# PaddlePaddle/PaddleNLP

Hardware: AMD Instinct MI355X
Metric: tokens_per_sec_whole_node_llama3_8b_pretrain (higher is better)
Workload: dtype bf16; 1 GPU; model=llama3-8b, global_batch=8, seq_len=4096, parallelism=single, recompute=False

## Files before the change

paddlenlp_amd/ops/csrc/flash_attn_bwd_v2.hip:

```cpp
#include "launchers.h"
#include "mfma.h"

#define FB2_WAVES 8
#define FB2_BLOCK (FB2_WAVES * 64)

template <int D, bool MASKED = false>
__global__ __launch_bounds__(FB2_BLOCK) void flash_bwd2_dq_kernel(
    const ushort_t* __restrict__ q, const ushort_t* __restrict__ k,
    const ushort_t* __restrict__ v, const ushort_t* __restrict__ dout,
    const float* __restrict__ lse, const float* __restrict__ delta,
    ushort_t* __restrict__ dq, const int* __restrict__ startend,
    FlashStrides rs,
    int B, int Sq, int Skv, int Hq, int Hk, float scale, int causal) {
    static_assert(D == 128, "the dual-use image is laid out for 128-column tiles");
    constexpr int BLKN = 64;
    constexpr int DSTEPS = D / 16;
    constexpr int NDT = D / 32;
    constexpr int BLKM = FB2_WAVES * 32;

    __shared__ __attribute__((aligned(16))) ushort_t kv_lds[2][2][BLKN * D];
    __shared__ int se_lds[3][MASKED ? BLKN : 1];

    const int tid = threadIdx.x;
    const int wave = __builtin_amdgcn_readfirstlane(tid >> 6);
    const int lane = tid & 63;
    const int l32 = lane & 31;
    const int hi = lane >> 5;

    int qt, bh;
    xcd_grouped_tile<FA_ORDER_W, false>(qt, bh);
    const int b = bh / Hq, hq = bh % Hq;
    const int hk = hq / (Hq / Hk);
    const int q_base = qt * BLKM;
    const int qw = q_base + wave * 32;
    const int qg = qw + l32;
    const int causal_off = Skv - Sq;

    const long long q_row_stride = rs.q;
    const long long kv_row_stride = rs.kv;
    const long long do_row_stride = (long long)Hq * D;
    const ushort_t* q_ptr = q + (long long)b * Sq * q_row_stride + (long long)hq * D;
    const ushort_t* do_ptr = dout + ((long long)b * Sq * Hq + hq) * D;
    const ushort_t* k_ptr = k + (long long)b * Skv * kv_row_stride + (long long)hk * D;
    const ushort_t* v_ptr = v + (long long)b * Skv * kv_row_stride + (long long)hk * D;

    frag8 aq[DSTEPS], ado[DSTEPS];
    float lse_q = INFINITY, dl_q = 0.f;
    if (qg < Sq) {
#pragma unroll
        for (int kk = 0; kk < DSTEPS; kk++) {
            aq[kk] = *reinterpret_cast<const frag8*>(
                q_ptr + (long long)qg * q_row_stride + kk * 16 + hi * 8);
            ado[kk] = *reinterpret_cast<const frag8*>(
                do_ptr + (long long)qg * do_row_stride + kk * 16 + hi * 8);
        }
        lse_q = lse[((long long)b * Hq + hq) * Sq + qg];
        dl_q = delta[((long long)b * Hq + hq) * Sq + qg];
    } else {
#pragma unroll
        for (int kk = 0; kk < DSTEPS; kk++) { aq[kk] = frag8{0}; ado[kk] = frag8{0}; }
    }

    f32x16 acc_dq[NDT];
#pragma unroll
    for (int n = 0; n < NDT; n++)
#pragma unroll
        for (int r = 0; r < 16; r++) acc_dq[n][r] = 0.f;

    int n_kv_tiles = (Skv + BLKN - 1) / BLKN;
    if (causal) {
        int max_kv = q_base + BLKM - 1 + causal_off;
        int lim = (max_kv + BLKN) / BLKN;
        n_kv_tiles = min(n_kv_tiles, max(lim, 0));
    }

    auto issue_tile = [&](int kv_base, int buf) {
        const int ln = fresh_lane_id();
#pragma unroll
        for (int i = 0; i < 2; i++) {
            const int piece = wave * 2 + i;
            const int src_row = min(kv_base + img_fill_row(piece, ln), Skv - 1);
            const long long off = (long long)src_row * kv_row_stride +
                                  img_fill_chunk(piece, ln) * 8;
            lds_dma16(k_ptr + off, &kv_lds[buf][0][piece * 512]);
            lds_dma16(v_ptr + off, &kv_lds[buf][1][piece * 512]);
        }
    };
    auto issue_bounds = [&](int tile, int slot) {
        if (MASKED && wave == 0) {
            const int ln = fresh_lane_id();
            lds_dma4(startend + (long long)b * Skv + min(tile * BLKN + ln, Skv - 1),
                     &se_lds[slot][0]);
        }
    };
    auto tile_se_max = [&](int slot) -> int {
        int v = se_lds[slot][lane];
#pragma unroll
        for (int off = 32; off; off >>= 1)
            v = max(v, __shfl_xor(v, off, 64));
        return __builtin_amdgcn_readfirstlane(v);
    };

#pragma unroll
    for (int kk = 0; kk < DSTEPS; kk++)
        asm volatile("" :: "v"(aq[kk]), "v"(ado[kk]));
    asm volatile("" :: "v"(lse_q), "v"(dl_q));
    if (n_kv_tiles > 0) {
        issue_tile(0, 0);
        issue_bounds(0, 0);
        if (n_kv_tiles > 1) issue_bounds(1, 1);
    }
    int se_max_cur = 0x7fffffff;
    int se_slot = 0;

    for (int kvt = 0; kvt < n_kv_tiles; kvt++) {
        const int kv_base = kvt * BLKN;
        const int cur = kvt & 1;
        lds_dma_wait_all();
        __syncthreads();
        const int se_slot_next = (se_slot == 2) ? 0 : se_slot + 1;
        if (MASKED && kvt == 0) se_max_cur = tile_se_max(0);
        int se_max_next = 0x7fffffff;
        if (kvt + 1 < n_kv_tiles) {
            bool stage_skip = false;
            if (MASKED) {
                se_max_next = tile_se_max(se_slot_next);
                stage_skip = (q_base >= se_max_next);
            }
            if (!stage_skip) issue_tile(kv_base + BLKN, cur ^ 1);
            if (kvt + 2 < n_kv_tiles)
                issue_bounds(kvt + 2, (se_slot_next == 2) ? 0 : se_slot_next + 1);
        }
        const ushort_t* k_img = kv_lds[cur][0];
        const ushort_t* v_img = kv_lds[cur][1];
        const int lane_t = fresh_lane_id();

        bool wave_skip =
            causal && (kv_base > qw + 31 + causal_off);
        if (MASKED && qw >= se_max_cur) wave_skip = true;

        auto process_sub = [&](int sub) {
            f32x16 st, dp;
#pragma unroll
            for (int r = 0; r < 16; r++) { st[r] = 0.f; dp[r] = 0.f; }
            __builtin_amdgcn_s_setprio(1);
#pragma unroll
            for (int kk = 0; kk < DSTEPS; kk++) {
                frag8 ak = img_row_frag(k_img, sub * 32 + l32, kk, hi);
                frag8 av = img_row_frag(v_img, sub * 32 + l32, kk, hi);
                st = mfma32(ak, aq[kk], st);
                dp = mfma32(av, ado[kk], dp);
            }
            __builtin_amdgcn_s_setprio(0);

#pragma unroll
            for (int r = 0; r < 16; r++) {
                int row = sub * 32 + crow32(r, hi);
                int kvg = kv_base + row;
                bool vis = (kvg < Skv) && (qg < Sq) &&
                           (!causal || kvg <= qg + causal_off);
                if (MASKED) vis = vis && (qg < se_lds[se_slot][row]);
                float p = vis ? __expf(st[r] * scale - lse_q) : 0.f;
                st[r] = p * (dp[r] - dl_q) * scale;
            }

            __builtin_amdgcn_s_setprio(1);
#pragma unroll
            for (int ksl = 0; ksl < 2; ksl++) {
                const int ks = sub * 2 + ksl;
                frag8 ads = t12_convert(st, ksl * 8);
#pragma unroll
                for (int n = 0; n < NDT; n++) {
                    frag8 bkf = img_tr_frag(k_img, ks, n, lane_t);
                    acc_dq[n] = mfma32(ads, bkf, acc_dq[n]);
                }
            }
            __builtin_amdgcn_s_setprio(0);
        };

        if (!wave_skip) {
            process_sub(0);
            process_sub(1);
        }
        if (MASKED) se_max_cur = se_max_next;
        se_slot = se_slot_next;
    }

#pragma unroll
    for (int r = 0; r < 16; r++) {
        int qrow = qw + crow32(r, hi);
        if (qrow >= Sq) continue;
        ushort_t* dqr = dq + ((long long)b * Sq + qrow) * rs.dq + (long long)hq * D;
#pragma unroll
        for (int n = 0; n < NDT; n++)
            dqr[n * 32 + l32] = f32_to_bf16(acc_dq[n][r]);
    }
}

template <int D, bool MASKED = false>
__global__ __launch_bounds__(FB2_BLOCK, 1) void flash_bwd2_dkv_kernel(
    const ushort_t* __restrict__ q, const ushort_t* __restrict__ k,
    const ushort_t* __restrict__ v, const ushort_t* __restrict__ dout,
    const float* __restrict__ lse, const float* __restrict__ delta,
    ushort_t* __restrict__ dk, ushort_t* __restrict__ dv,
    const int* __restrict__ startend,
    FlashStrides rs,
    int B, int Sq, int Skv, int Hq, int Hk, float scale, int causal) {
    static_assert(D == 128, "the dual-use image is laid out for 128-column tiles");
    constexpr int BLKQ = 64;
    constexpr int DSTEPS = D / 16;
    constexpr int NDT = D / 32;
    constexpr int BLKKV = FB2_WAVES * 32;

    __shared__ __attribute__((aligned(16))) ushort_t qd_lds[2][2][BLKQ * D];
    __shared__ float ld_lds[2][2][BLKQ];

    const int tid = threadIdx.x;
    const int wave = __builtin_amdgcn_readfirstlane(tid >> 6);
    const int lane = tid & 63;
    const int l32 = lane & 31;
    const int hi = lane >> 5;

    int kvt, bh;
    xcd_grouped_tile<FA_ORDER_W, true>(kvt, bh);
    const int b = bh / Hk, hk = bh % Hk;
    const int G = Hq / Hk;
    const int kv_base = kvt * BLKKV;
    const int kvw = kv_base + wave * 32;
    const int kvg_lane = kvw + l32;
    const int causal_off = Skv - Sq;
    __shared__ int blk_max_lds[MASKED ? FB2_WAVES : 1];
    int kv_end_lane = 0x7fffffff;
    int wave_max_end = 0x7fffffff;
    if (MASKED) {
        kv_end_lane = (kvg_lane < Skv)
            ? startend[(long long)b * Skv + kvg_lane] : 0;
        wave_max_end = kv_end_lane;
#pragma unroll
        for (int off = 32; off; off >>= 1)
            wave_max_end = max(wave_max_end,
                               __shfl_xor(wave_max_end, off, 64));
        wave_max_end = __builtin_amdgcn_readfirstlane(wave_max_end);
        if (lane == 0) blk_max_lds[wave] = wave_max_end;
    }

    const long long do_row_stride = (long long)Hq * D;
    const ushort_t* k_ptr = k + (long long)b * Skv * rs.kv + (long long)hk * D;
    const ushort_t* v_ptr = v + (long long)b * Skv * rs.kv + (long long)hk * D;

    frag8 bk[DSTEPS], bv[DSTEPS];
    if (kvg_lane < Skv) {
#pragma unroll
        for (int kk = 0; kk < DSTEPS; kk++) {
            bk[kk] = *reinterpret_cast<const frag8*>(
                k_ptr + (long long)kvg_lane * rs.kv + kk * 16 + hi * 8);
            bv[kk] = *reinterpret_cast<const frag8*>(
                v_ptr + (long long)kvg_lane * rs.kv + kk * 16 + hi * 8);
        }
    } else {
#pragma unroll
        for (int kk = 0; kk < DSTEPS; kk++) { bk[kk] = frag8{0}; bv[kk] = frag8{0}; }
    }

    f32x16 acc_dk[NDT], acc_dv[NDT];
#pragma unroll
    for (int n = 0; n < NDT; n++)
#pragma unroll
        for (int r = 0; r < 16; r++) { acc_dk[n][r] = 0.f; acc_dv[n][r] = 0.f; }

    int qt0 = 0;
    if (causal) qt0 = max(0, (kv_base - causal_off) / BLKQ);
    int qt_end = (Sq + BLKQ - 1) / BLKQ;
    if (MASKED) {
        __syncthreads();
        int block_max_end = blk_max_lds[0];
#pragma unroll
        for (int w = 1; w < FB2_WAVES; w++)
            block_max_end = max(block_max_end, blk_max_lds[w]);
        block_max_end = __builtin_amdgcn_readfirstlane(block_max_end);
        if (block_max_end < Sq)
            qt_end = (max(block_max_end, 0) + BLKQ - 1) / BLKQ;
    }
    const int n_tiles = G * max(qt_end - qt0, 0);

    auto issue_tile = [&](int g, int qt, int buf) {
        const int hq = hk * G + g;
        const long long do_off = ((long long)b * Sq * Hq + hq) * D;
        const long long q_off = (long long)b * Sq * rs.q + (long long)hq * D;
        const int q_tb = qt * BLKQ;
        const int ln = fresh_lane_id();
#pragma unroll
        for (int i = 0; i < 2; i++) {
            const int piece = wave * 2 + i;
            const int src_row = min(q_tb + img_fill_row(piece, ln), Sq - 1);
            const int chunk = img_fill_chunk(piece, ln) * 8;
            lds_dma16(q + (q_off + (long long)src_row * rs.q + chunk),
                      &qd_lds[buf][0][piece * 512]);
            lds_dma16(dout + (do_off + (long long)src_row * do_row_stride + chunk),
                      &qd_lds[buf][1][piece * 512]);
        }
        if (wave < 2) {
            const float* row = (wave == 0 ? lse : delta) +
                               ((long long)b * Hq + hq) * Sq;
            lds_dma4(row + min(q_tb + ln, Sq - 1), &ld_lds[buf][wave][0]);
        }
    };

    int g_next = 0, qt_next = qt0;
    auto advance_next = [&]() {
        if (++qt_next == qt_end) { qt_next = qt0; g_next++; }
    };
#pragma unroll
    for (int kk = 0; kk < DSTEPS; kk++)
        asm volatile("" :: "v"(bk[kk]), "v"(bv[kk]));
    if (n_tiles > 0) { issue_tile(g_next, qt_next, 0); advance_next(); }

    int qt = qt0;
    for (int t = 0; t < n_tiles; t++) {
        const int cur = t & 1;
        lds_dma_wait_all();
        __syncthreads();
        if (t + 1 < n_tiles) { issue_tile(g_next, qt_next, cur ^ 1); advance_next(); }

        const int q_tb = qt * BLKQ;
        const ushort_t* q_img = qd_lds[cur][0];
        const ushort_t* do_img = qd_lds[cur][1];
        const int lane_t = fresh_lane_id();
        bool wave_skip =
            causal && (q_tb + BLKQ - 1 + causal_off < kvw);
        if (MASKED && q_tb >= wave_max_end) wave_skip = true;

        if (!wave_skip) {
#pragma unroll 1
            for (int sub = 0; sub < 2; sub++) {
                f32x16 st, dp;
#pragma unroll
                for (int r = 0; r < 16; r++) { st[r] = 0.f; dp[r] = 0.f; }
                __builtin_amdgcn_s_setprio(1);
#pragma unroll
                for (int kk = 0; kk < DSTEPS; kk++) {
                    frag8 aqf = img_row_frag(q_img, sub * 32 + l32, kk, hi);
                    frag8 adf = img_row_frag(do_img, sub * 32 + l32, kk, hi);
                    st = mfma32(aqf, bk[kk], st);
                    dp = mfma32(adf, bv[kk], dp);
                }
                __builtin_amdgcn_s_setprio(0);

#pragma unroll
                for (int r = 0; r < 16; r++) {
                    int qrow = sub * 32 + crow32(r, hi);
                    int qgl = q_tb + qrow;
                    float ls = ld_lds[cur][0][qrow];
                    float dl = ld_lds[cur][1][qrow];
                    bool vis = (qgl < Sq) && (kvg_lane < Skv) &&
                               (!causal || kvg_lane <= qgl + causal_off);
                    if (MASKED) vis = vis && (qgl < kv_end_lane);
                    float p = (vis && ls != INFINITY)
                                  ? __expf(st[r] * scale - ls) : 0.f;
                    st[r] = p;
                    dp[r] = p * (dp[r] - dl) * scale;
                }

                __builtin_amdgcn_s_setprio(1);
#pragma unroll
                for (int ksl = 0; ksl < 2; ksl++) {
                    const int ks = sub * 2 + ksl;
                    frag8 apt = t12_convert(st, ksl * 8);
                    frag8 ads = t12_convert(dp, ksl * 8);
#pragma unroll
                    for (int n = 0; n < NDT; n++) {
                        frag8 bdo = img_tr_frag(do_img, ks, n, lane_t);
                        frag8 bq = img_tr_frag(q_img, ks, n, lane_t);
                        acc_dv[n] = mfma32(apt, bdo, acc_dv[n]);
                        acc_dk[n] = mfma32(ads, bq, acc_dk[n]);
                    }
                }
                __builtin_amdgcn_s_setprio(0);
            }
        }
        if (++qt == qt_end) qt = qt0;
    }

#pragma unroll
    for (int r = 0; r < 16; r++) {
        int kvr = kvw + crow32(r, hi);
        if (kvr >= Skv) continue;
        long long base = ((long long)b * Skv + kvr) * rs.dkv + (long long)hk * D;
#pragma unroll
        for (int n = 0; n < NDT; n++) {
            dk[base + n * 32 + l32] = f32_to_bf16(acc_dk[n][r]);
            dv[base + n * 32 + l32] = f32_to_bf16(acc_dv[n][r]);
        }
    }
}

__global__ __launch_bounds__(64) void lds_image_probe(
    const ushort_t* __restrict__ X, ushort_t* __restrict__ out_row,
    ushort_t* __restrict__ out_tr) {
    __shared__ __attribute__((aligned(16))) ushort_t img[64 * 128];
    const int lane = threadIdx.x;
    const int l32 = lane & 31, hi = lane >> 5;
#pragma unroll 1
    for (int piece = 0; piece < 16; piece++)
        lds_dma16(X + img_fill_row(piece, lane) * 128 + img_fill_chunk(piece, lane) * 8,
                  &img[piece * 512]);
    lds_dma_wait_all();
    __syncthreads();
    for (int sub = 0; sub < 2; sub++)
        for (int kk = 0; kk < 8; kk++) {
            frag8 f = img_row_frag(img, sub * 32 + l32, kk, hi);
            *reinterpret_cast<frag8*>(
                out_row + (sub * 32 + l32) * 128 + kk * 16 + hi * 8) = f;
        }
    for (int ks = 0; ks < 4; ks++)
        for (int n = 0; n < 4; n++) {
            frag8 f = img_tr_frag(img, ks, n, lane);
#pragma unroll
            for (int j = 0; j < 8; j++)
                out_tr[(ks * 16 + hi * 8 + j) * 128 + n * 32 + l32] = (ushort_t)f[j];
        }
}

void launch_lds_image_probe(const void* X, void* out_row, void* out_tr,
                            hipStream_t stream) {
    hipLaunchKernelGGL(lds_image_probe, dim3(1), dim3(64), 0, stream,
                       (const ushort_t*)X, (ushort_t*)out_row, (ushort_t*)out_tr);
}

bool launch_flash_bwd2(const void* dout, const void* q, const void* k, const void* v,
                       const void* o, const float* lse, float* delta,
                       void* dq, void* dk, void* dv,
                       int B, int Sq, int Skv, int Hq, int Hk, int D,
                       float scale, bool causal, hipStream_t stream, int parts,
                       const FlashStrides* strides) {
    if (D != 128 || (Hq % Hk) != 0) return false;
    const FlashStrides rs = strides ? *strides : flash_contiguous_strides(Hq, Hk, D);
    if (!flash_dma_aligned(q, rs.q) || !flash_dma_aligned(k, rs.kv) ||
        !flash_dma_aligned(v, rs.kv) || !flash_dma_aligned(dout, Hq * D))
        return false;
    if (parts & FLASH_BWD_DELTA)
        launch_flash_bwd_delta(dout, o, delta, B, Sq, Hq, D, stream);
    if (parts & FLASH_BWD_DQ) {
        dim3 gq((Sq + 255) / 256, B * Hq);
        hipLaunchKernelGGL((flash_bwd2_dq_kernel<128, false>), gq, dim3(FB2_BLOCK), 0, stream,
                           (const ushort_t*)q, (const ushort_t*)k, (const ushort_t*)v,
                           (const ushort_t*)dout, lse, delta, (ushort_t*)dq,
                           (const int*)nullptr, rs,
                           B, Sq, Skv, Hq, Hk, scale, causal ? 1 : 0);
    }
    if (parts & FLASH_BWD_DKV) {
        dim3 gkv((Skv + 255) / 256, B * Hk);
        hipLaunchKernelGGL((flash_bwd2_dkv_kernel<128, false>), gkv, dim3(FB2_BLOCK), 0, stream,
                           (const ushort_t*)q, (const ushort_t*)k, (const ushort_t*)v,
                           (const ushort_t*)dout, lse, delta, (ushort_t*)dk, (ushort_t*)dv,
                           (const int*)nullptr, rs,
                           B, Sq, Skv, Hq, Hk, scale, causal ? 1 : 0);
    }
    return true;
}

bool launch_flash_bwd2_mask(const void* dout, const void* q, const void* k,
                            const void* v, const void* o, const float* lse,
                            float* delta, void* dq, void* dk, void* dv,
                            const int* startend,
                            int B, int Sq, int Skv, int Hq, int Hk, int D,
                            float scale, hipStream_t stream,
                            const FlashStrides* strides) {
    if (D != 128 || (Hq % Hk) != 0) return false;
    const FlashStrides rs = strides ? *strides : flash_contiguous_strides(Hq, Hk, D);
    if (!flash_dma_aligned(q, rs.q) || !flash_dma_aligned(k, rs.kv) ||
        !flash_dma_aligned(v, rs.kv) || !flash_dma_aligned(dout, Hq * D))
        return false;
    launch_flash_bwd_delta(dout, o, delta, B, Sq, Hq, D, stream);
    dim3 gq((Sq + 255) / 256, B * Hq);
    hipLaunchKernelGGL((flash_bwd2_dq_kernel<128, true>), gq, dim3(FB2_BLOCK), 0, stream,
                       (const ushort_t*)q, (const ushort_t*)k, (const ushort_t*)v,
                       (const ushort_t*)dout, lse, delta, (ushort_t*)dq, startend, rs,
                       B, Sq, Skv, Hq, Hk, scale, 1);
    dim3 gkv((Skv + 255) / 256, B * Hk);
    hipLaunchKernelGGL((flash_bwd2_dkv_kernel<128, true>), gkv, dim3(FB2_BLOCK), 0, stream,
                       (const ushort_t*)q, (const ushort_t*)k, (const ushort_t*)v,
                       (const ushort_t*)dout, lse, delta, (ushort_t*)dk, (ushort_t*)dv,
                       startend, rs, B, Sq, Skv, Hq, Hk, scale, 1);
    return true;
}
```

paddlenlp_amd/ops/csrc/flash_attn_v2.hip:

```cpp
#include "launchers.h"
#include "mfma.h"

#define FA2_WAVES 8
#define FA2_BLOCK (FA2_WAVES * 64)
#define FA2_BLKN 64
#define FA2_QW 32
#define FA2_BLKM (FA2_WAVES * FA2_QW)
#define DEFER_THR 8.0f

__global__ void mfma32_layout_probe(const ushort_t* A, const ushort_t* B, float* C) {
    int l = threadIdx.x;
    int l32 = l & 31, hi = l >> 5;
    frag8 a, b;
#pragma unroll
    for (int j = 0; j < 8; j++) {
        a[j] = (short)A[l32 * 16 + hi * 8 + j];
        b[j] = (short)B[(hi * 8 + j) * 32 + l32];
    }
    f32x16 c;
#pragma unroll
    for (int r = 0; r < 16; r++) c[r] = 0.f;
    c = mfma32(a, b, c);
#pragma unroll
    for (int r = 0; r < 16; r++) C[crow32(r, hi) * 32 + l32] = c[r];
}

__global__ void permlane_probe(int* out0, int* out1) {
    int l = threadIdx.x;
    auto r = __builtin_amdgcn_permlane32_swap((unsigned)l, (unsigned)(1000 + l),
                                              false, false);
    out0[l] = (int)r[0];
    out1[l] = (int)r[1];
}

template <int D, bool MASKED = false>
__global__ __launch_bounds__(FA2_BLOCK) void flash_fwd2_kernel(
    const ushort_t* __restrict__ q,
    const ushort_t* __restrict__ k,
    const ushort_t* __restrict__ v,
    ushort_t* __restrict__ o,
    float* __restrict__ lse,
    const int* __restrict__ startend,
    FlashStrides rs,
    int B, int Sq, int Skv, int Hq, int Hk, float scale, int causal) {
    static_assert(D == 128, "the dual-use image is laid out for 128-column tiles");
    constexpr int DSTEPS = D / 16;
    constexpr int NDT = D / 32;
    constexpr int KVT = FA2_BLKN / 32;

    __shared__ __attribute__((aligned(16))) ushort_t kv_lds[2][2][FA2_BLKN * D];
    __shared__ int se_lds[3][MASKED ? FA2_BLKN : 1];

    const int tid = threadIdx.x;
    const int wave = __builtin_amdgcn_readfirstlane(tid >> 6);
    const int lane = tid & 63;
    const int l32 = lane & 31;
    const int hi = lane >> 5;

    int qt, bh;
    xcd_grouped_tile<FA_ORDER_W, false>(qt, bh);
    const int b = bh / Hq, hq = bh % Hq;
    const int hk = hq / (Hq / Hk);
    const int q_base = qt * FA2_BLKM;
    const int qw = q_base + wave * FA2_QW;
    const int qg = qw + l32;
    const int causal_off = Skv - Sq;

    const long long q_row_stride = rs.q;
    const long long kv_row_stride = rs.kv;
    const long long o_row_stride = (long long)Hq * D;
    const ushort_t* q_ptr = q + (long long)b * Sq * q_row_stride + (long long)hq * D;
    const ushort_t* k_ptr = k + (long long)b * Skv * kv_row_stride + (long long)hk * D;
    const ushort_t* v_ptr = v + (long long)b * Skv * kv_row_stride + (long long)hk * D;

    frag8 aq[DSTEPS];
    if (qg < Sq) {
#pragma unroll
        for (int kk = 0; kk < DSTEPS; kk++)
            aq[kk] = *reinterpret_cast<const frag8*>(
                q_ptr + (long long)qg * q_row_stride + kk * 16 + hi * 8);
    } else {
#pragma unroll
        for (int kk = 0; kk < DSTEPS; kk++) aq[kk] = frag8{0};
    }

    float m_run = -INFINITY, l_run = 0.f;
    f32x16 acc_o[NDT];
#pragma unroll
    for (int n = 0; n < NDT; n++)
#pragma unroll
        for (int r = 0; r < 16; r++) acc_o[n][r] = 0.f;

    int n_kv_tiles = (Skv + FA2_BLKN - 1) / FA2_BLKN;
    if (causal) {
        int max_kv = q_base + FA2_BLKM - 1 + causal_off;
        int lim = (max_kv + FA2_BLKN) / FA2_BLKN;
        n_kv_tiles = min(n_kv_tiles, max(lim, 0));
    }

    auto issue_tile = [&](int kv_base, int buf) {
        const int ln = fresh_lane_id();
#pragma unroll
        for (int i = 0; i < 2; i++) {
            const int piece = wave * 2 + i;
            const int src_row = min(kv_base + img_fill_row(piece, ln), Skv - 1);
            const long long off = (long long)src_row * kv_row_stride +
                                  img_fill_chunk(piece, ln) * 8;
            lds_dma16(k_ptr + off, &kv_lds[buf][0][piece * 512]);
            lds_dma16(v_ptr + off, &kv_lds[buf][1][piece * 512]);
        }
    };
    auto issue_bounds = [&](int tile, int slot) {
        if (MASKED && wave == 0) {
            const int ln = fresh_lane_id();
            lds_dma4(startend + (long long)b * Skv + min(tile * FA2_BLKN + ln, Skv - 1),
                     &se_lds[slot][0]);
        }
    };
    auto tile_bounds = [&](int slot, int& mn_out) -> int {
        int mx = se_lds[slot][lane], mn = mx;
#pragma unroll
        for (int off = 32; off; off >>= 1) {
            mx = max(mx, __shfl_xor(mx, off, 64));
            mn = min(mn, __shfl_xor(mn, off, 64));
        }
        mn_out = __builtin_amdgcn_readfirstlane(mn);
        return __builtin_amdgcn_readfirstlane(mx);
    };

#pragma unroll
    for (int kk = 0; kk < DSTEPS; kk++) asm volatile("" :: "v"(aq[kk]));
    if (n_kv_tiles > 0) {
        issue_tile(0, 0);
        issue_bounds(0, 0);
        if (n_kv_tiles > 1) issue_bounds(1, 1);
    }
    int se_min_cur = 0, se_max_cur = 0x7fffffff;
    int se_slot = 0;

    for (int kvt = 0; kvt < n_kv_tiles; kvt++) {
        const int kv_base = kvt * FA2_BLKN;
        const int cur = kvt & 1;
        lds_dma_wait_all();
        __syncthreads();
        const int se_slot_next = (se_slot == 2) ? 0 : se_slot + 1;
        if (MASKED && kvt == 0) se_max_cur = tile_bounds(0, se_min_cur);
        int se_min_next = 0, se_max_next = 0x7fffffff;
        if (kvt + 1 < n_kv_tiles) {
            bool stage_skip = false;
            if (MASKED) {
                se_max_next = tile_bounds(se_slot_next, se_min_next);
                stage_skip = (q_base >= se_max_next);
            }
            if (!stage_skip) issue_tile(kv_base + FA2_BLKN, cur ^ 1);
            if (kvt + 2 < n_kv_tiles)
                issue_bounds(kvt + 2, (se_slot_next == 2) ? 0 : se_slot_next + 1);
        }
        const ushort_t* k_img = kv_lds[cur][0];
        const ushort_t* v_img = kv_lds[cur][1];
        const int lane_t = fresh_lane_id();

        bool wave_skip =
            causal && (kv_base > qw + FA2_QW - 1 + causal_off);
        if (MASKED && qw >= se_max_cur) wave_skip = true;

        f32x16 st[KVT];
        if (!wave_skip) {
#pragma unroll
            for (int nt = 0; nt < KVT; nt++)
#pragma unroll
                for (int r = 0; r < 16; r++) st[nt][r] = 0.f;
            __builtin_amdgcn_s_setprio(1);
#pragma unroll
            for (int kk = 0; kk < DSTEPS; kk++) {
#pragma unroll
                for (int nt = 0; nt < KVT; nt++) {
                    frag8 ak = img_row_frag(k_img, nt * 32 + l32, kk, hi);
                    st[nt] = mfma32(ak, aq[kk], st[nt]);
                }
            }
            __builtin_amdgcn_s_setprio(0);

            const bool full_tile =
                (kv_base + FA2_BLKN <= Skv) &&
                (!causal || (kv_base + FA2_BLKN - 1 <= qw + causal_off)) &&
                (!MASKED || (qw + FA2_QW - 1 < se_min_cur));
            if (full_tile) {
#pragma unroll
                for (int nt = 0; nt < KVT; nt++)
#pragma unroll
                    for (int r = 0; r < 16; r++) st[nt][r] *= scale;
            } else {
#pragma unroll
                for (int nt = 0; nt < KVT; nt++)
#pragma unroll
                    for (int r = 0; r < 16; r++) {
                        int row = nt * 32 + crow32(r, hi);
                        int kvg = kv_base + row;
                        bool vis = (kvg < Skv) &&
                                   (!causal || kvg <= qg + causal_off);
                        if (MASKED) vis = vis && (qg < se_lds[se_slot][row]);
                        st[nt][r] = vis ? st[nt][r] * scale : -INFINITY;
                    }
            }

            float pm = -INFINITY;
#pragma unroll
            for (int nt = 0; nt < KVT; nt++)
#pragma unroll
                for (int r = 0; r < 16; r++) pm = fmaxf(pm, st[nt][r]);
            {
                union { float f; unsigned u; } x{pm};
                auto rr = __builtin_amdgcn_permlane32_swap(x.u, x.u, false, false);
                union { unsigned u; float f; } a{rr[0]}, c{rr[1]};
                pm = fmaxf(a.f, c.f);
            }

            bool grew = pm > m_run + DEFER_THR ||
                        (m_run == -INFINITY && pm > -INFINITY);
            if (__any(grew)) {
                float m_new = fmaxf(m_run, pm);
                float alpha = (m_run == -INFINITY)
                                  ? 0.f
                                  : __expf(m_run - m_new);
                if (m_new == -INFINITY) alpha = 1.f;
                l_run *= alpha;
                m_run = m_new;
#pragma unroll
                for (int r = 0; r < 16; r++) {
                    float ar = __shfl(alpha, crow32(r, hi), 64);
#pragma unroll
                    for (int n = 0; n < NDT; n++) acc_o[n][r] *= ar;
                }
            }

            float ps = 0.f;
#pragma unroll
            for (int nt = 0; nt < KVT; nt++)
#pragma unroll
                for (int r = 0; r < 16; r++) {
                    float s = st[nt][r];
                    float p = (s == -INFINITY) ? 0.f : __expf(s - m_run);
                    st[nt][r] = p;
                    ps += p;
                }
            {
                union { float f; unsigned u; } x{ps};
                auto rr = __builtin_amdgcn_permlane32_swap(x.u, x.u, false, false);
                union { unsigned u; float f; } a{rr[0]}, c{rr[1]};
                ps = a.f + c.f;
            }
            l_run += ps;

            __builtin_amdgcn_s_setprio(1);
#pragma unroll
            for (int ks = 0; ks < FA2_BLKN / 16; ks++) {
                frag8 pa = t12_convert(st[ks >> 1], (ks & 1) * 8);
#pragma unroll
                for (int n = 0; n < NDT; n++) {
                    frag8 bv = img_tr_frag(v_img, ks, n, lane_t);
                    acc_o[n] = mfma32(pa, bv, acc_o[n]);
                }
            }
            __builtin_amdgcn_s_setprio(0);
        }

        if (MASKED) { se_max_cur = se_max_next; se_min_cur = se_min_next; }
        se_slot = se_slot_next;
    }

    float inv_l = (l_run > 0.f) ? 1.0f / l_run : 0.f;
#pragma unroll
    for (int r = 0; r < 16; r++) {
        int qrow = qw + crow32(r, hi);
        if (qrow >= Sq) continue;
        float il = __shfl(inv_l, crow32(r, hi), 64);
        ushort_t* orow = o + ((long long)b * Sq + qrow) * o_row_stride + (long long)hq * D;
#pragma unroll
        for (int n = 0; n < NDT; n++)
            orow[n * 32 + l32] = f32_to_bf16(acc_o[n][r] * il);
    }
    if (hi == 0 && qg < Sq) {
        float lv = (l_run > 0.f) ? (m_run + __logf(l_run)) : -INFINITY;
        lse[((long long)b * Hq + hq) * Sq + qg] = lv;
    }
}

void launch_mfma32_probe(const void* A, const void* B, float* C, hipStream_t stream) {
    hipLaunchKernelGGL(mfma32_layout_probe, dim3(1), dim3(64), 0, stream,
                       (const ushort_t*)A, (const ushort_t*)B, C);
}

void launch_permlane_probe(int* out0, int* out1, hipStream_t stream) {
    hipLaunchKernelGGL(permlane_probe, dim3(1), dim3(64), 0, stream, out0, out1);
}

bool launch_flash_fwd2(const void* q, const void* k, const void* v, void* o,
                       float* lse, int B, int Sq, int Skv, int Hq, int Hk,
                       int D, float scale, bool causal, hipStream_t stream,
                       const FlashStrides* strides) {
    if (D != 128 || (Hq % Hk) != 0) return false;
    const FlashStrides rs = strides ? *strides : flash_contiguous_strides(Hq, Hk, D);
    if (!flash_dma_aligned(k, rs.kv) || !flash_dma_aligned(v, rs.kv)) return false;
    dim3 grid((Sq + FA2_BLKM - 1) / FA2_BLKM, B * Hq);
    hipLaunchKernelGGL((flash_fwd2_kernel<128, false>), grid, dim3(FA2_BLOCK), 0, stream,
                       (const ushort_t*)q, (const ushort_t*)k, (const ushort_t*)v,
                       (ushort_t*)o, lse, (const int*)nullptr, rs,
                       B, Sq, Skv, Hq, Hk, scale, causal ? 1 : 0);
    return true;
}

bool launch_flash_fwd2_mask(const void* q, const void* k, const void* v,
                            void* o, float* lse, const int* startend,
                            int B, int Sq, int Skv, int Hq, int Hk,
                            int D, float scale, hipStream_t stream,
                            const FlashStrides* strides) {
    if (D != 128 || (Hq % Hk) != 0) return false;
    const FlashStrides rs = strides ? *strides : flash_contiguous_strides(Hq, Hk, D);
    if (!flash_dma_aligned(k, rs.kv) || !flash_dma_aligned(v, rs.kv)) return false;
    dim3 grid((Sq + FA2_BLKM - 1) / FA2_BLKM, B * Hq);
    hipLaunchKernelGGL((flash_fwd2_kernel<128, true>), grid, dim3(FA2_BLOCK), 0,
                       stream, (const ushort_t*)q, (const ushort_t*)k,
                       (const ushort_t*)v, (ushort_t*)o, lse, startend, rs,
                       B, Sq, Skv, Hq, Hk, scale, 1);
    return true;
}
```

paddlenlp_amd/ops/csrc/mfma.h:

```cpp
#pragma once

#include "common.h"

typedef short8v frag8;

__device__ __forceinline__ f32x4 mfma16(frag8 a, frag8 b, f32x4 c) {
    return __builtin_amdgcn_mfma_f32_16x16x32_bf16(a, b, c, 0, 0, 0);
}

__device__ __forceinline__ f32x16 mfma32(frag8 a, frag8 b, f32x16 c) {
    return __builtin_amdgcn_mfma_f32_32x32x16_bf16(a, b, c, 0, 0, 0);
}

__device__ __forceinline__ int crow32(int r, int hi) {
    return (r & 3) + 8 * (r >> 2) + 4 * hi;
}

template <int LD>
__device__ __forceinline__ char* swz(ushort_t* base, int row, int col_elem) {
    return reinterpret_cast<char*>(base) +
           (((row * LD + col_elem) * 2) ^ ((row & 7) << 4));
}

__device__ __forceinline__ unsigned pack_bf16(float a, float b) {
    return (unsigned)f32_to_bf16(a) | ((unsigned)f32_to_bf16(b) << 16);
}

__device__ __forceinline__ frag8 t12_convert(const f32x16& p, int rb) {
    unsigned w[4];
    {
        unsigned lo0 = pack_bf16(p[rb + 0], p[rb + 1]);
        unsigned hi0 = pack_bf16(p[rb + 4], p[rb + 5]);
        auto rr = __builtin_amdgcn_permlane32_swap(lo0, hi0, false, false);
        w[0] = rr[0]; w[2] = rr[1];
    }
    {
        unsigned lo1 = pack_bf16(p[rb + 2], p[rb + 3]);
        unsigned hi1 = pack_bf16(p[rb + 6], p[rb + 7]);
        auto rr = __builtin_amdgcn_permlane32_swap(lo1, hi1, false, false);
        w[1] = rr[0]; w[3] = rr[1];
    }
    frag8 f;
#pragma unroll
    for (int j = 0; j < 4; j++) {
        f[j * 2] = (short)(w[j] & 0xffff);
        f[j * 2 + 1] = (short)(w[j] >> 16);
    }
    return f;
}

__device__ __forceinline__ int img_off(int row, int ch) {
    return 2048 * (row >> 3) + 512 * (ch >> 2) + 64 * (row & 7) +
           16 * ((ch & 3) ^ ((row >> 2) & 3));
}

typedef short short4v __attribute__((ext_vector_type(4)));
typedef __attribute__((address_space(3))) short4v lds_short4v;

__device__ __forceinline__ int img_fill_row(int piece, int lane) {
    return 8 * (piece >> 1) + ((lane >> 2) & 7);
}
__device__ __forceinline__ int img_fill_chunk(int piece, int lane) {
    const int row = img_fill_row(piece, lane);
    return 4 * (2 * (piece & 1) + (lane >> 5)) + ((lane & 3) ^ ((row >> 2) & 3));
}
__device__ __forceinline__ unsigned lds_addr(const void* p) {
    return (unsigned)(unsigned long long)p;
}
__device__ __forceinline__ void lds_dma16(const void* src, const void* lds_dst) {
    unsigned keep;
    asm volatile("s_mov_b32 %0, m0\n\ts_mov_b32 m0, %2\n\ts_nop 0\n\t"
                 "global_load_lds_dwordx4 %1, off\n\ts_mov_b32 m0, %0"
                 : "=&s"(keep) : "v"(src), "s"(lds_addr(lds_dst)) : "memory");
}
__device__ __forceinline__ void lds_dma4(const void* src, const void* lds_dst) {
    unsigned keep;
    asm volatile("s_mov_b32 %0, m0\n\ts_mov_b32 m0, %2\n\ts_nop 0\n\t"
                 "global_load_lds_dword %1, off\n\ts_mov_b32 m0, %0"
                 : "=&s"(keep) : "v"(src), "s"(lds_addr(lds_dst)) : "memory");
}
__device__ __forceinline__ void lds_dma_wait_all() {
    asm volatile("s_waitcnt vmcnt(0)" ::: "memory");
}

__device__ __forceinline__ frag8 img_row_frag(const ushort_t* img, int row, int kk, int hi) {
    return *reinterpret_cast<const frag8*>(
        reinterpret_cast<const char*>(img) + img_off(row, kk * 2 + hi));
}

__device__ __forceinline__ frag8 img_tr_frag(const ushort_t* img, int ks, int n, int lane) {
    const int i = lane & 15, qq = i >> 2, p = i & 3;
    const int hi = lane >> 5;
    const int c0 = n * 4 + ((lane >> 4) & 1) * 2 + (p >> 1);
    const char* base = reinterpret_cast<const char*>(img) + 8 * (p & 1);
    frag8 f;
#pragma unroll
    for (int jj = 0; jj < 2; jj++) {
        const int row = ks * 16 + hi * 8 + jj * 4 + qq;
        short4v t = __builtin_amdgcn_ds_read_tr16_b64_v4i16(
            (lds_short4v*)(base + img_off(row, c0)));
#pragma unroll
        for (int e = 0; e < 4; e++) f[jj * 4 + e] = t[e];
    }
    return f;
}

__device__ __forceinline__ int fresh_lane_id() {
    int ln;
    asm volatile("v_mbcnt_lo_u32_b32 %0, -1, 0\n\tv_mbcnt_hi_u32_b32 %0, -1, %0"
                 : "=v"(ln));
    return ln;
}

#define FA_ORDER_W 4
template <int W, bool ASCENDING>
__device__ __forceinline__ void xcd_grouped_tile(int& tile, int& bh) {
    const int T = gridDim.x;
    if ((gridDim.y & 7) != 0) {
        tile = blockIdx.x;
        bh = blockIdx.y;
        return;
    }
    const int flat = blockIdx.x + T * blockIdx.y;
    const int idx = flat >> 3;
    const int hp = gridDim.y >> 3;
    const int grp = idx / (W * T);
    const int rem = idx - grp * (W * T);
    const int wg = min(W, hp - grp * W);
    const int rank = rem / wg;
    tile = ASCENDING ? rank : T - 1 - rank;
    bh = (flat & 7) * hp + grp * W + (rem - rank * wg);
}
```

Before: 21950 tokens/s.

## Streamline flash attention softmax with full-tile mask skipping and packed bf16 conversion

Forward and both backward flash attention kernels now compute exp unconditionally with fused multiply-add and apply the visibility mask only on tiles that are not fully visible. Fully visible tiles are detected using per-tile min bounds for the masked variant. The scale multiply moves after the max reduction, which uses v_max3. LSE/delta loads in the dkv kernel are vectorized, and bf16 packing uses a native vector convert. Opaque asm barriers and an s_nop fence control scheduling, but they may constrain the compiler. The exp is now evaluated on masked entries too, relying on later zeroing.

```diff
diff --git a/paddlenlp_amd/ops/csrc/flash_attn_bwd_v2.hip b/paddlenlp_amd/ops/csrc/flash_attn_bwd_v2.hip
--- a/paddlenlp_amd/ops/csrc/flash_attn_bwd_v2.hip
+++ b/paddlenlp_amd/ops/csrc/flash_attn_bwd_v2.hip
@@ -93,12 +93,15 @@
                      &se_lds[slot][0]);
         }
     };
-    auto tile_se_max = [&](int slot) -> int {
-        int v = se_lds[slot][lane];
-#pragma unroll
-        for (int off = 32; off; off >>= 1)
-            v = max(v, __shfl_xor(v, off, 64));
-        return __builtin_amdgcn_readfirstlane(v);
+    auto tile_bounds = [&](int slot, int& mn_out) -> int {
+        int mx = se_lds[slot][lane], mn = mx;
+#pragma unroll
+        for (int off = 32; off; off >>= 1) {
+            mx = max(mx, __shfl_xor(mx, off, 64));
+            mn = min(mn, __shfl_xor(mn, off, 64));
+        }
+        mn_out = __builtin_amdgcn_readfirstlane(mn);
+        return __builtin_amdgcn_readfirstlane(mx);
     };
 
 #pragma unroll
@@ -110,7 +113,7 @@
         issue_bounds(0, 0);
         if (n_kv_tiles > 1) issue_bounds(1, 1);
     }
-    int se_max_cur = 0x7fffffff;
+    int se_min_cur = 0, se_max_cur = 0x7fffffff;
     int se_slot = 0;
 
     for (int kvt = 0; kvt < n_kv_tiles; kvt++) {
@@ -119,12 +122,12 @@
         lds_dma_wait_all();
         __syncthreads();
         const int se_slot_next = (se_slot == 2) ? 0 : se_slot + 1;
-        if (MASKED && kvt == 0) se_max_cur = tile_se_max(0);
-        int se_max_next = 0x7fffffff;
+        if (MASKED && kvt == 0) se_max_cur = tile_bounds(0, se_min_cur);
+        int se_min_next = 0, se_max_next = 0x7fffffff;
         if (kvt + 1 < n_kv_tiles) {
             bool stage_skip = false;
             if (MASKED) {
-                se_max_next = tile_se_max(se_slot_next);
+                se_max_next = tile_bounds(se_slot_next, se_min_next);
                 stage_skip = (q_base >= se_max_next);
             }
             if (!stage_skip) issue_tile(kv_base + BLKN, cur ^ 1);
@@ -153,15 +156,26 @@
             }
             __builtin_amdgcn_s_setprio(0);
 
+            const int kv_sub = kv_base + sub * 32;
+            const bool full_sub =
+                (kv_sub + 32 <= Skv) && (qw + 31 < Sq) &&
+                (!causal || (kv_sub + 31 <= qw + causal_off)) &&
+                (!MASKED || (qw + 31 < se_min_cur));
 #pragma unroll
             for (int r = 0; r < 16; r++) {
-                int row = sub * 32 + crow32(r, hi);
-                int kvg = kv_base + row;
-                bool vis = (kvg < Skv) && (qg < Sq) &&
-                           (!causal || kvg <= qg + causal_off);
-                if (MASKED) vis = vis && (qg < se_lds[se_slot][row]);
-                float p = vis ? __expf(st[r] * scale - lse_q) : 0.f;
-                st[r] = p * (dp[r] - dl_q) * scale;
+                float p = __expf(__builtin_fmaf(st[r], scale, -lse_q));
+                st[r] = sm_opaque(p * (dp[r] - dl_q) * scale);
+            }
+            if (!full_sub) {
+#pragma unroll
+                for (int r = 0; r < 16; r++) {
+                    int row = sub * 32 + crow32(r, hi);
+                    int kvg = kv_base + row;
+                    bool vis = (kvg < Skv) && (qg < Sq) &&
+                               (!causal || kvg <= qg + causal_off);
+                    if (MASKED) vis = vis && (qg < se_lds[se_slot][row]);
+                    st[r] = vis ? st[r] : 0.f;
+                }
             }
 
             __builtin_amdgcn_s_setprio(1);
@@ -182,7 +196,7 @@
             process_sub(0);
             process_sub(1);
         }
-        if (MASKED) se_max_cur = se_max_next;
+        if (MASKED) { se_max_cur = se_max_next; se_min_cur = se_min_next; }
         se_slot = se_slot_next;
     }
 
@@ -213,7 +227,7 @@
     constexpr int BLKKV = FB2_WAVES * 32;
 
     __shared__ __attribute__((aligned(16))) ushort_t qd_lds[2][2][BLKQ * D];
-    __shared__ float ld_lds[2][2][BLKQ];
+    __shared__ __attribute__((aligned(16))) float ld_lds[2][2][BLKQ];
 
     const int tid = threadIdx.x;
     const int wave = __builtin_amdgcn_readfirstlane(tid >> 6);
@@ -232,15 +246,21 @@
     __shared__ int blk_max_lds[MASKED ? FB2_WAVES : 1];
     int kv_end_lane = 0x7fffffff;
     int wave_max_end = 0x7fffffff;
+    int wave_min_end = 0x7fffffff;
     if (MASKED) {
         kv_end_lane = (kvg_lane < Skv)
             ? startend[(long long)b * Skv + kvg_lane] : 0;
         wave_max_end = kv_end_lane;
-#pragma unroll
-        for (int off = 32; off; off >>= 1)
+        wave_min_end = kv_end_lane;
+#pragma unroll
+        for (int off = 32; off; off >>= 1) {
             wave_max_end = max(wave_max_end,
                                __shfl_xor(wave_max_end, off, 64));
+            wave_min_end = min(wave_min_end,
+                               __shfl_xor(wave_min_end, off, 64));
+        }
         wave_max_end = __builtin_amdgcn_readfirstlane(wave_max_end);
+        wave_min_end = __builtin_amdgcn_readfirstlane(wave_min_end);
         if (lane == 0) blk_max_lds[wave] = wave_max_end;
     }
 
@@ -325,7 +345,6 @@
         const int q_tb = qt * BLKQ;
         const ushort_t* q_img = qd_lds[cur][0];
         const ushort_t* do_img = qd_lds[cur][1];
-        const int lane_t = fresh_lane_id();
         bool wave_skip =
             causal && (q_tb + BLKQ - 1 + causal_off < kvw);
         if (MASKED && q_tb >= wave_max_end) wave_skip = true;
@@ -346,33 +365,54 @@
                 }
                 __builtin_amdgcn_s_setprio(0);
 
-#pragma unroll
-                for (int r = 0; r < 16; r++) {
-                    int qrow = sub * 32 + crow32(r, hi);
-                    int qgl = q_tb + qrow;
-                    float ls = ld_lds[cur][0][qrow];
-                    float dl = ld_lds[cur][1][qrow];
-                    bool vis = (qgl < Sq) && (kvg_lane < Skv) &&
-                               (!causal || kvg_lane <= qgl + causal_off);
-                    if (MASKED) vis = vis && (qgl < kv_end_lane);
-                    float p = (vis && ls != INFINITY)
-                                  ? __expf(st[r] * scale - ls) : 0.f;
-                    st[r] = p;
-                    dp[r] = p * (dp[r] - dl) * scale;
-                }
-
+                const int q_sub = q_tb + sub * 32;
+                const bool full_sub =
+                    (q_sub + 32 <= Sq) && (kvw + 32 <= Skv) &&
+                    (!causal || (kvw + 31 <= q_sub + causal_off)) &&
+                    (!MASKED || (q_sub + 31 < wave_min_end));
+#pragma unroll
+                for (int g = 0; g < 4; g++) {
+                    const int row0 = sub * 32 + 8 * g + 4 * hi;
+                    const f32x4 ls4 = *reinterpret_cast<const f32x4*>(&ld_lds[cur][0][row0]);
+                    const f32x4 dl4 = *reinterpret_cast<const f32x4*>(&ld_lds[cur][1][row0]);
+#pragma unroll
+                    for (int j = 0; j < 4; j++) {
+                        const int r = 4 * g + j;
+                        float p = sm_opaque(__expf(__builtin_fmaf(st[r], scale, -ls4[j])));
+                        st[r] = p;
+                        dp[r] = sm_opaque(p * (dp[r] - dl4[j]) * scale);
+                    }
+                }
+                if (!full_sub) {
+#pragma unroll
+                    for (int r = 0; r < 16; r++) {
+                        int qgl = q_sub + crow32(r, hi);
+                        bool vis = (qgl < Sq) && (kvg_lane < Skv) &&
+                                   (!causal || kvg_lane <= qgl + causal_off);
+                        if (MASKED) vis = vis && (qgl < kv_end_lane);
+                        st[r] = vis ? st[r] : 0.f;
+                        dp[r] = vis ? dp[r] : 0.f;
+                    }
+                }
+
+                frag8 apt[2], ads[2];
+#pragma unroll
+                for (int ksl = 0; ksl < 2; ksl++) {
+                    apt[ksl] = t12_convert(st, ksl * 8);
+                    ads[ksl] = t12_convert(dp, ksl * 8);
+                }
+                asm volatile("" : "+v"(apt[0]), "+v"(apt[1]), "+v"(ads[0]), "+v"(ads[1]));
+                const int lane_t = fresh_lane_id();
                 __builtin_amdgcn_s_setprio(1);
 #pragma unroll
                 for (int ksl = 0; ksl < 2; ksl++) {
                     const int ks = sub * 2 + ksl;
-                    frag8 apt = t12_convert(st, ksl * 8);
-                    frag8 ads = t12_convert(dp, ksl * 8);
 #pragma unroll
                     for (int n = 0; n < NDT; n++) {
                         frag8 bdo = img_tr_frag(do_img, ks, n, lane_t);
                         frag8 bq = img_tr_frag(q_img, ks, n, lane_t);
-                        acc_dv[n] = mfma32(apt, bdo, acc_dv[n]);
-                        acc_dk[n] = mfma32(ads, bq, acc_dk[n]);
+                        acc_dv[n] = mfma32(apt[ksl], bdo, acc_dv[n]);
+                        acc_dk[n] = mfma32(ads[ksl], bq, acc_dk[n]);
                     }
                 }
                 __builtin_amdgcn_s_setprio(0);
diff --git a/paddlenlp_amd/ops/csrc/flash_attn_v2.hip b/paddlenlp_amd/ops/csrc/flash_attn_v2.hip
--- a/paddlenlp_amd/ops/csrc/flash_attn_v2.hip
+++ b/paddlenlp_amd/ops/csrc/flash_attn_v2.hip
@@ -181,16 +181,14 @@
             }
             __builtin_amdgcn_s_setprio(0);
 
+            static_assert(KVT == 2, "sm_fence below covers exactly two S tiles");
+            sm_fence(st[0], st[1]);
+
             const bool full_tile =
                 (kv_base + FA2_BLKN <= Skv) &&
                 (!causal || (kv_base + FA2_BLKN - 1 <= qw + causal_off)) &&
                 (!MASKED || (qw + FA2_QW - 1 < se_min_cur));
-            if (full_tile) {
-#pragma unroll
-                for (int nt = 0; nt < KVT; nt++)
-#pragma unroll
-                    for (int r = 0; r < 16; r++) st[nt][r] *= scale;
-            } else {
+            if (!full_tile) {
 #pragma unroll
                 for (int nt = 0; nt < KVT; nt++)
 #pragma unroll
@@ -200,15 +198,14 @@
                         bool vis = (kvg < Skv) &&
                                    (!causal || kvg <= qg + causal_off);
                         if (MASKED) vis = vis && (qg < se_lds[se_slot][row]);
-                        st[nt][r] = vis ? st[nt][r] * scale : -INFINITY;
+                        st[nt][r] = vis ? st[nt][r] : -INFINITY;
                     }
             }
 
             float pm = -INFINITY;
 #pragma unroll
-            for (int nt = 0; nt < KVT; nt++)
-#pragma unroll
-                for (int r = 0; r < 16; r++) pm = fmaxf(pm, st[nt][r]);
+            for (int nt = 0; nt < KVT; nt++) pm = sm_tile_max(pm, st[nt]);
+            pm *= scale;
             {
                 union { float f; unsigned u; } x{pm};
                 auto rr = __builtin_amdgcn_permlane32_swap(x.u, x.u, false, false);
@@ -234,13 +231,13 @@
                 }
             }
 
+            const float m_eff = (m_run == -INFINITY) ? 0.f : m_run;
             float ps = 0.f;
 #pragma unroll
             for (int nt = 0; nt < KVT; nt++)
 #pragma unroll
                 for (int r = 0; r < 16; r++) {
-                    float s = st[nt][r];
-                    float p = (s == -INFINITY) ? 0.f : __expf(s - m_run);
+                    float p = sm_opaque(__expf(sm_opaque(st[nt][r] * scale) - m_eff));
                     st[nt][r] = p;
                     ps += p;
                 }
diff --git a/paddlenlp_amd/ops/csrc/mfma.h b/paddlenlp_amd/ops/csrc/mfma.h
--- a/paddlenlp_amd/ops/csrc/mfma.h
+++ b/paddlenlp_amd/ops/csrc/mfma.h
@@ -16,14 +16,35 @@
     return (r & 3) + 8 * (r >> 2) + 4 * hi;
 }
 
+__device__ __forceinline__ float sm_opaque(float x) {
+    asm("" : "+v"(x));
+    return x;
+}
+__device__ __forceinline__ void sm_fence(f32x16& a, f32x16& b) {
+    asm volatile("s_nop 11" : "+v"(a), "+v"(b));
+}
+__device__ __forceinline__ float sm_max3(float a, float b, float c) {
+    float d;
+    asm("v_max3_f32 %0, %1, %2, %3" : "=v"(d) : "v"(a), "v"(b), "v"(c));
+    return d;
+}
+__device__ __forceinline__ float sm_tile_max(float m, const f32x16& s) {
+#pragma unroll
+    for (int r = 0; r < 16; r += 2) m = sm_max3(m, s[r], s[r + 1]);
+    return m;
+}
+
 template <int LD>
 __device__ __forceinline__ char* swz(ushort_t* base, int row, int col_elem) {
     return reinterpret_cast<char*>(base) +
            (((row * LD + col_elem) * 2) ^ ((row & 7) << 4));
 }
 
+typedef __bf16 bf16x2v __attribute__((ext_vector_type(2)));
 __device__ __forceinline__ unsigned pack_bf16(float a, float b) {
-    return (unsigned)f32_to_bf16(a) | ((unsigned)f32_to_bf16(b) << 16);
+    union { bf16x2v h; unsigned u; } r;
+    r.h = __builtin_convertvector(f32x2{a, b}, bf16x2v);
+    return r.u;
 }
 
 __device__ __forceinline__ frag8 t12_convert(const f32x16& p, int rb) {
```

Result: faster. 22790 tokens/s (median of 6 runs) (+3.8%).
